# pujariaditya/WaveVerify

Measured on AMD Instinct MI355X. Metric: clips/sec embed+detect, 1s@16kHz bs=256, higher is better.
Workload: dtype f32; 1 GPU; embed_detect: 256 clips x 1 s @ 16 kHz per GPU (BASELINE.json configs[1]), seeded random weights; batch_per_gpu=256, global_batch=256, clip_samples=16000, parallelism=dp1 (independent clip shards, no data-path collective)

## Files before the change

### waveverify_amd/csrc/wv_rb.hip

```cpp
#include <atomic>
#include <string>

#include "wv_dev.h"

namespace wv {

namespace {

template <int NT> struct RbVec;
template <> struct RbVec<4> { typedef f32x4 type; };
template <> struct RbVec<2> { typedef f32x2 type; };

constexpr int RB_OOB = 0x7f000000;
#ifndef RB_CFG64
#define RB_CFG64 RB<64, 2, 4, 2, 1>
#endif
#ifndef RB_CFG96
#define RB_CFG96 RB<96, 4, 2, 3, 3>
#endif
#ifndef RB_CFG128
#define RB_CFG128 RB<128, 2, 4, 2, 4>
#endif
#ifndef RB_CFG192
#define RB_CFG192 RB<192, 2, 2, 3, 2>
#endif
#ifndef RB_PD
#define RB_PD 3
#endif
#ifndef RB_AD
#define RB_AD 3
#endif

#ifdef RB_STAMP
#define RB_T(i) do { const unsigned long long t_ = __builtin_amdgcn_s_memtime(); ph[i] += t_ - tprev; tprev = t_; } while (0)
#else
#define RB_T(i) do {} while (0)
#endif

template <int C_, int NG_, int NT_, int WPS_, int PARTS_>
struct RB {
    static constexpr int C = C_, NG = NG_, NT = NT_, WPS = WPS_, PARTS = PARTS_;
    static constexpr int WM = C / 32, NWAVES = WM * NG, NTHREADS = 64 * NWAVES;
    static constexpr int GS = 32 * NT - 4;
    static constexpr int WD = NG * GS + 4;
    static constexpr int TTO = WD - 8;
    static constexpr int LD = WD;
    static constexpr int NCH = C / 16;
    static constexpr int W4 = WD / 4, P4 = C * W4;
    static constexpr int RPI = 64 / W4;
    static constexpr int NI = (C / RPI + NWAVES - 1) / NWAVES;
    static constexpr size_t SMEM = ((size_t)C * LD + 2 * C * 8) * sizeof(float);
    static_assert(C % 32 == 0 && WD % 4 == 0 && (NT == 2 || NT == 4) && NTHREADS >= 2 * C && RPI >= 1 && C % RPI == 0 && 16 % RPI == 0 &&
                  PARTS >= 1 && NCH % PARTS == 0, "geometry");
    static_assert((2 * NCH) % (RB_AD + 1) == 0, "the A ring must close over a tile");
};

#define RB_BARRIER()                                             \
    do {                                                         \
        asm volatile("s_waitcnt lgkmcnt(0)" ::: "memory");       \
        __builtin_amdgcn_s_barrier();                            \
        asm volatile("" ::: "memory");                           \
    } while (0)

__device__ __forceinline__ float rb_dpp_next(float v) {
    return __builtin_bit_cast(float, __builtin_amdgcn_update_dpp(0, __builtin_bit_cast(int, v), 0x130, 0xf, 0xf, true));
}

__device__ __forceinline__ f32x2 rb_pair_next(f32x2 v) { return f32x2{rb_dpp_next(v.x), rb_dpp_next(v.y)}; }
template <int NT>
__device__ __forceinline__ void rb_stencil2(const f32x16 (&acc)[NT], int r, const float* tp, f32x2 (&y)[NT]) {
    const f32x4 q0 = *reinterpret_cast<const f32x4*>(tp), q1 = *reinterpret_cast<const f32x4*>(tp + 4), q2 = *reinterpret_cast<const f32x4*>(tp + 8);
    const f32x2 w[5] = {{q0.x, q0.y}, {q0.z, q0.w}, {q1.x, q1.y}, {q1.z, q1.w}, {q2.x, q2.y}};
    const f32x2 bb{q2.z, q2.w};
    f32x2 col[NT + 4];
#pragma unroll
    for (int e = 0; e < NT; ++e) col[e] = f32x2{acc[e][r], acc[e][r + 1]};
    if constexpr (NT == 4) {
#pragma unroll
        for (int e = 0; e < 4; ++e) col[4 + e] = rb_pair_next(col[e]);
    } else {
        col[2] = rb_pair_next(col[0]); col[3] = rb_pair_next(col[1]);
        col[4] = rb_pair_next(col[2]); col[5] = rb_pair_next(col[3]);
    }
#pragma unroll
    for (int e = 0; e < NT; ++e) {
        f32x2 v = bb;
#pragma unroll
        for (int i = 0; i < 5; ++i) v = __builtin_elementwise_fma(w[i], col[e + i], v);
        y[e] = v;
    }
}

template <class R, int G0, class LoadA, class AtChunk>
__device__ __forceinline__ void rb_gemm(f32x16 (&acc)[R::NT], f32x4 (&ar)[RB_AD + 1][2], const float* Bf, LoadA&& load_a,
                                        const __amdgpu_buffer_rsrc_t& rw, const __amdgpu_buffer_rsrc_t& rw_next, AtChunk&& at_chunk) {
    typedef typename RbVec<R::NT>::type bvec;
    constexpr int NS = 8 * R::NCH, PD = RB_PD, NB = PD + 1, AD = RB_AD, NA = AD + 1;
    bvec bq[NB];
    auto row_of = [](int s) { return 16 * (s >> 3) + ((s & 7) < 4 ? (s & 7) : 4 + (s & 7)); };
#pragma unroll
    for (int s = 0; s < PD; ++s) bq[s % NB] = *reinterpret_cast<const bvec*>(Bf + row_of(s) * R::LD);
#pragma unroll
    for (int s = 0; s < NS; ++s) {
        const int c = s >> 3, j = s & 7;
        if (j == 0) {
            if (c > 0) at_chunk(c);
            if (c + AD < R::NCH) load_a(rw, c + AD, ar[(G0 + c + AD) % NA]);
            else load_a(rw_next, c + AD - R::NCH, ar[(G0 + c + AD) % NA]);
        }
        if (s + PD < NS) bq[(s + PD) % NB] = *reinterpret_cast<const bvec*>(Bf + row_of(s + PD) * R::LD);
        const f32x4 av = ar[(G0 + c) % NA][j >> 2];
        const float a = av[j & 3];
        const bvec bv = bq[s % NB];
#pragma unroll
        for (int e = 0; e < R::NT; ++e) acc[e] = __builtin_amdgcn_mfma_f32_32x32x2f32(a, bv[e], acc[e], 0, 0, 0);
        __builtin_amdgcn_sched_barrier(0);
    }
}

template <class R, int OUT>
__global__ __launch_bounds__(R::NTHREADS) __attribute__((amdgpu_waves_per_eu(R::WPS, R::WPS))) void rb_kernel(RbArgs p) {
    extern __shared__ __attribute__((aligned(16))) float smem[];
    typedef typename RbVec<R::NT>::type ovec;
    typedef unsigned uvec __attribute__((ext_vector_type(R::NT)));
    constexpr int NT = R::NT, C = R::C, LD = R::LD, NCH = R::NCH, AD = RB_AD, NA = AD + 1;
    float* S = smem;
    float* tab = smem + C * LD;
    const int tid = threadIdx.x, lane = tid & 63;
    const int wave = __builtin_amdgcn_readfirstlane(tid >> 6);
    const int strip = wave % R::WM, grp = wave / R::WM;
    const int h = lane >> 5, q = lane & 31;
    const int T = p.T, ntiles = p.ntiles, num_t = p.num_t;
    const int row_bytes = T * 4, clip_bytes = C * T * 4;

    for (int i = tid; i < C * 8; i += R::NTHREADS) {
        const int m = i >> 3, j = i & 7;
        if (j < 6) {
            const int d = (m >> 1) * 12 + 2 * (j < 5 ? j : 5) + (m & 1);
            tab[d] = p.tab1[i]; tab[C * 8 + d] = p.tab2[i];
        }
    }

    constexpr int MP = (C + M_ALIGN - 1) / M_ALIGN * M_ALIGN;
    const __amdgpu_buffer_rsrc_t rW1 = uniform_rsrc(p.pw1.wq, NCH * 4 * MP * 16);
    const __amdgpu_buffer_rsrc_t rW2 = uniform_rsrc(p.pw2.wq, NCH * 4 * MP * 16);
    const int avoff = (h * MP + 32 * strip + q) * 16;
    f32x4 ar[NA][2];
    auto load_a = [&](const __amdgpu_buffer_rsrc_t& rw, int c, f32x4 (&dst)[2]) {
        dst[0] = __builtin_bit_cast(f32x4, __builtin_amdgcn_raw_buffer_load_b128(rw, avoff, c * 4 * MP * 16, 0));
        dst[1] = __builtin_bit_cast(f32x4, __builtin_amdgcn_raw_buffer_load_b128(rw, avoff, (c * 4 + 2) * MP * 16, 0));
    };

    const int co = R::GS * grp + NT * q;
    const bool own = NT * q < R::GS && co < R::TTO;
    const bool uw = NT * q < R::GS;
    const int row0 = 32 * strip + 4 * h;
    const float* Bf = S + co + 4 * h * LD;
    const float* Wrow1 = tab + (row0 / 2) * 12;
    const float* Wrow2 = Wrow1 + C * 8;
    float* Urow = S + row0 * LD + co;
    float* Xrow = Urow + 8;
    const bool hthread = tid < 2 * C;
    const int hrow = tid >> 1, hpc = tid & 1;

    ovec X[16];
    const int xrow = lane / R::W4, xc4 = lane - xrow * R::W4;
    const bool xlane = lane < R::RPI * R::W4;
    auto refill = [&](int t, int row0_, int row1_) {
        if (t < 0) return;
        const int b = t / num_t, tt = t - b * num_t;
        const int tw0 = tt * R::TTO - 8;
        const __amdgpu_buffer_rsrc_t rX = uniform_rsrc(p.X + (size_t)b * C * T, clip_bytes);
        const int tx = tw0 + 4 * xc4;
        const int vo = (tx >= 0 && tx < T) ? (xrow * T + tx) * 4 : RB_OOB;
        if (xlane) {
#pragma unroll
            for (int i = 0; i < R::NI; ++i) {
                const int rb = i * R::NWAVES + wave;
                const int r_ = rb * R::RPI, so = r_ * row_bytes;
                float* dst = S + r_ * LD;
                if (r_ >= row0_ && r_ < row1_)
                    __builtin_amdgcn_raw_ptr_buffer_load_lds(rX, (__attribute__((address_space(3))) void*)dst, 16, vo, so, 0, 0);
            }
        }
    };
    auto x_off = [&](int to0) { const int t = to0 + co; return (own && t < T) ? (row0 * T + t) * 4 : RB_OOB; };
    const bool h0own = (OUT & 4) && co >= 8 && co < R::WD && (NT * q < R::GS || (grp == R::NG - 1 && NT * q < R::GS + 4));
    const bool u_own = (OUT & 4) && uw && co >= 4 && co < R::WD - 4;
    auto sv_off = [&](bool mine, int t) { return (mine && t < T) ? (row0 * T + t) * 4 : RB_OOB; };
    const float oscale = p.out_scale_ptr ? p.out_scale * p.out_scale_ptr[0] : p.out_scale;

    int tile = blockIdx.x;
    if (tile >= ntiles) return;
    refill(tile, 0, C);
#pragma unroll
    for (int c = 0; c < AD; ++c) load_a(rW1, c, ar[c % NA]);
    asm volatile("s_waitcnt vmcnt(0)" ::: "memory");
    RB_BARRIER();

#ifdef RB_STAMP
    unsigned long long ph[9] = {0, 0, 0, 0, 0, 0, 0, 0, 0}, tprev = __builtin_amdgcn_s_memtime();
#endif
    for (; tile < ntiles; tile += gridDim.x) {
        const int b = tile / num_t, tt = tile - b * num_t;
        const int to0 = tt * R::TTO;
        if (hthread) {
            f32x4* hp = reinterpret_cast<f32x4*>(S + hrow * LD + 4 * hpc);
            f32x4 v = *hp;
            v.x = elu1(v.x * p.pre_scale); v.y = elu1(v.y * p.pre_scale); v.z = elu1(v.z * p.pre_scale); v.w = elu1(v.w * p.pre_scale);
            *hp = v;
        }
        if (own) {
#pragma unroll
            for (int r = 0; r < 16; ++r) X[r] = *reinterpret_cast<const ovec*>(Xrow + ((r & 3) + 8 * (r >> 2)) * LD);
#pragma unroll
            for (int r = 0; r < 16; ++r) {
                ovec v;
#pragma unroll
                for (int e = 0; e < NT; ++e) v[e] = elu1(X[r][e] * p.pre_scale);
                *reinterpret_cast<ovec*>(Xrow + ((r & 3) + 8 * (r >> 2)) * LD) = v;
            }
        }
        RB_T(0);
        RB_BARRIER();
        RB_T(1);
        f32x16 acc[NT];
#pragma unroll
        for (int e = 0; e < NT; ++e)
#pragma unroll
            for (int r = 0; r < 16; ++r) acc[e][r] = 0.f;
        rb_gemm<R, 0>(acc, ar, Bf, load_a, rW1, rW2, [](int) {});
        RB_T(2);
        RB_BARRIER();
        RB_T(3);
        {
            const size_t bo1 = (size_t)b * C * T;
            const __amdgpu_buffer_rsrc_t rH0 = uniform_rsrc((OUT & 4) ? p.sv_h0 + bo1 : p.X, (OUT & 4) ? clip_bytes : 0);
            const __amdgpu_buffer_rsrc_t rU = uniform_rsrc((OUT & 4) ? p.sv_u + bo1 : p.X, (OUT & 4) ? clip_bytes : 0);
            const int vh0 = sv_off(h0own, to0 - 8 + co), vu = sv_off(u_own, to0 - 4 + co);
#pragma unroll
            for (int r = 0; r < 16; r += 2) {
                const int cr = (r & 3) + 8 * (r >> 2);
                f32x2 y2[NT];
                rb_stencil2<NT>(acc, r, Wrow1 + (cr / 2) * 12, y2);
#pragma unroll
                for (int k = 0; k < 2; ++k) {
                    ovec uv;
#pragma unroll
                    for (int e = 0; e < NT; ++e) uv[e] = elu1(y2[e][k] * 1.f);
                    if (uw) *reinterpret_cast<ovec*>(Urow + (cr + k) * LD) = uv;
                    if constexpr ((OUT & 4) != 0) {
                        ovec hv, ur;
#pragma unroll
                        for (int e = 0; e < NT; ++e) { hv[e] = acc[e][r + k]; ur[e] = y2[e][k]; }
                        const int o0 = vh0 == RB_OOB ? RB_OOB : vh0 + (cr + k) * row_bytes, o1 = vu == RB_OOB ? RB_OOB : vu + (cr + k) * row_bytes;
                        if constexpr (NT == 4) {
                            __builtin_amdgcn_raw_buffer_store_b128(__builtin_bit_cast(uvec, hv), rH0, o0, 0, 0);
                            __builtin_amdgcn_raw_buffer_store_b128(__builtin_bit_cast(uvec, ur), rU, o1, 0, 0);
                        } else {
                            __builtin_amdgcn_raw_buffer_store_b64(__builtin_bit_cast(uvec, hv), rH0, o0, 0, 0);
                            __builtin_amdgcn_raw_buffer_store_b64(__builtin_bit_cast(uvec, ur), rU, o1, 0, 0);
                        }
                    }
                }
                __builtin_amdgcn_sched_barrier(0);
            }
            if (tt == 0 && grp == 0 && NT * q < 4) {
                ovec z;
#pragma unroll
                for (int e = 0; e < NT; ++e) z[e] = 0.f;
#pragma unroll
                for (int r = 0; r < 16; ++r) *reinterpret_cast<ovec*>(Urow + ((r & 3) + 8 * (r >> 2)) * LD) = z;
            }
        }
        RB_T(4);
        RB_BARRIER();
        RB_T(5);
#pragma unroll
        for (int e = 0; e < NT; ++e)
#pragma unroll
            for (int r = 0; r < 16; ++r) acc[e][r] = 0.f;
        const int next = tile + gridDim.x < ntiles ? tile + gridDim.x : -1;
        rb_gemm<R, NCH>(acc, ar, Bf, load_a, rW2, rW1, [&](int c) {
            if (R::PARTS > 1 && c % (NCH / R::PARTS) == 0) {
                constexpr int per = NCH / R::PARTS;
                RB_BARRIER();
                refill(next, 16 * (c - per), 16 * c);
            }
        });
        RB_T(6);
        RB_BARRIER();
        RB_T(7);
        {
            const size_t bo = (size_t)b * C * T;
            const __amdgpu_buffer_rsrc_t rY = uniform_rsrc((OUT & 1) ? p.Y + bo : p.X, (OUT & 1) ? clip_bytes : 0);
            const __amdgpu_buffer_rsrc_t rA = uniform_rsrc((OUT & 2) ? p.Yact + bo : p.X, (OUT & 2) ? clip_bytes : 0);
            const int voff0 = x_off(to0);
            const __amdgpu_buffer_rsrc_t rH1 = uniform_rsrc((OUT & 4) ? p.sv_h1 + bo : p.X, (OUT & 4) ? clip_bytes : 0);
            const __amdgpu_buffer_rsrc_t rV = uniform_rsrc((OUT & 4) ? p.sv_v + bo : p.X, (OUT & 4) ? clip_bytes : 0);
            const int vh1 = sv_off(u_own, to0 - 4 + co);
            refill(next, R::PARTS > 1 ? 16 * (NCH - NCH / R::PARTS) : 0, C);
#pragma unroll
            for (int r = 0; r < 16; r += 2) {
                const int cr0 = (r & 3) + 8 * (r >> 2);
                f32x2 v2[NT];
                rb_stencil2<NT>(acc, r, Wrow2 + (cr0 / 2) * 12, v2);
#pragma unroll
                for (int k = 0; k < 2; ++k) {
                    const int cr = cr0 + k;
                    ovec y;
#pragma unroll
                    for (int e = 0; e < NT; ++e) y[e] = fmaf(v2[e][k], oscale, X[r + k][e]);
                    const int off = voff0 + cr * row_bytes;
                    if constexpr ((OUT & 4) != 0) {
                        ovec hv, vv;
#pragma unroll
                        for (int e = 0; e < NT; ++e) { hv[e] = acc[e][r + k]; vv[e] = v2[e][k]; }
                        const int o1 = vh1 == RB_OOB ? RB_OOB : vh1 + cr * row_bytes;
                        if constexpr (NT == 4) {
                            __builtin_amdgcn_raw_buffer_store_b128(__builtin_bit_cast(uvec, hv), rH1, o1, 0, 0);
                            __builtin_amdgcn_raw_buffer_store_b128(__builtin_bit_cast(uvec, vv), rV, off, 0, 0);
                        } else {
                            __builtin_amdgcn_raw_buffer_store_b64(__builtin_bit_cast(uvec, hv), rH1, o1, 0, 0);
                            __builtin_amdgcn_raw_buffer_store_b64(__builtin_bit_cast(uvec, vv), rV, off, 0, 0);
                        }
                    }
                    if constexpr ((OUT & 1) != 0) {
                        if constexpr (NT == 4) __builtin_amdgcn_raw_buffer_store_b128(__builtin_bit_cast(uvec, y), rY, off, 0, 0);
                        else __builtin_amdgcn_raw_buffer_store_b64(__builtin_bit_cast(uvec, y), rY, off, 0, 0);
                    }
                    if constexpr ((OUT & 2) != 0) {
                        ovec a;
#pragma unroll
                        for (int e = 0; e < NT; ++e) a[e] = elu1(y[e] * p.act_scale);
                        if constexpr (NT == 4) __builtin_amdgcn_raw_buffer_store_b128(__builtin_bit_cast(uvec, a), rA, off, 0, 0);
                        else __builtin_amdgcn_raw_buffer_store_b64(__builtin_bit_cast(uvec, a), rA, off, 0, 0);
                    }
                }
                __builtin_amdgcn_sched_barrier(0);
            }
        }
        RB_T(8);
        asm volatile("s_waitcnt vmcnt(%0)" :: "n"(16 * ((OUT & 1) + ((OUT >> 1) & 1) + ((OUT & 4) ? 2 : 0))) : "memory");
        RB_BARRIER();
    }
#ifdef RB_STAMP
    if (lane == 0 && (OUT & 1)) {
        asm volatile("s_waitcnt vmcnt(0)" ::: "memory");
        for (int i = 0; i < 9; ++i) p.Y[((size_t)blockIdx.x * R::NWAVES + wave) * 9 + i] = (float)ph[i];
    }
#endif
}

bool aligned16(const void* p) { return (reinterpret_cast<uintptr_t>(p) & 15) == 0; }

int cu_count() {
    static std::atomic<int> cached[32];
    int d = 0;
    (void)hipGetDevice(&d);
    d &= 31;
    int n = cached[d].load(std::memory_order_relaxed);
    if (n == 0) {
        hipDeviceProp_t pr;
        n = hipGetDeviceProperties(&pr, d) == hipSuccess && pr.multiProcessorCount > 0 ? pr.multiProcessorCount : 256;
        cached[d].store(n, std::memory_order_relaxed);
    }
    return n;
}

template <class R, int OUT>
hipError_t rb_launch(RbArgs a, hipStream_t s) {
    a.num_t = (a.T + R::TTO - 1) / R::TTO;
    const long long nt = (long long)a.num_t * a.B;
    if (nt > 0x7fffffffLL) return hipErrorInvalidValue;
    a.ntiles = (int)nt;
    static std::atomic<unsigned> attr{0};
    if (R::SMEM > 64 * 1024) {
        int d = 0; (void)hipGetDevice(&d);
        const unsigned bit = 1u << (d & 31);
        if (!(attr.load(std::memory_order_relaxed) & bit)) {
            hipError_t e = hipFuncSetAttribute(reinterpret_cast<const void*>(rb_kernel<R, OUT>),
                                               hipFuncAttributeMaxDynamicSharedMemorySize, (int)R::SMEM);
            if (e != hipSuccess) return e;
            attr.fetch_or(bit, std::memory_order_relaxed);
        }
    }
    const int per_cu = std::max(1, std::min((int)(160 * 1024 / R::SMEM), 4 * R::WPS / R::NWAVES));
    const int grid = (int)std::min<long long>(nt, (long long)cu_count() * per_cu);
    std::string name;
    if (prof::enabled()) name = std::string((OUT & 4) ? "resblock_train<" : "resblock<") + std::to_string(R::C) + "," + std::to_string(R::WD) + ">";
    const double C = a.C, Bd = a.B, T = a.T;
    prof::Scope ps(s, name.c_str(), 2.0 * 2.0 * Bd * C * (C * T + 5.0 * T),
                   4.0 * Bd * C * T * (1.0 + ((OUT & 1) ? 1.0 : 0.0) + ((OUT & 2) ? 1.0 : 0.0) + ((OUT & 4) ? 4.0 : 0.0)));
    hipLaunchKernelGGL((rb_kernel<R, OUT>), dim3((unsigned)grid), dim3(R::NTHREADS), R::SMEM, s, a);
    return hipGetLastError();
}

template <class R>
hipError_t rb_pick_out(const RbArgs& a, hipStream_t s) {
    if (a.sv_h0) return rb_launch<R, 5>(a, s);
    if (a.Y && a.Yact) return rb_launch<R, 3>(a, s);
    if (a.Y) return rb_launch<R, 1>(a, s);
    return rb_launch<R, 2>(a, s);
}

}

bool rb_supported(const RbArgs& a) {
    if (!(a.C == 64 || a.C == 96 || a.C == 128 || a.C == 192)) return false;
    if (!a.X || (!a.Y && !a.Yact) || a.T < 4 || (a.T & 3) || a.B < 1 || !a.pw1.wq || !a.pw2.wq || !a.tab1 || !a.tab2) return false;
    if (a.pw1.M != a.C || a.pw1.K != a.C || a.pw2.M != a.C || a.pw2.K != a.C) return false;
    if (a.pw1.Mp != round_up(a.C, M_ALIGN) || a.pw2.Mp != a.pw1.Mp) return false;
    if ((long long)a.C * a.T * 4 >= RB_OOB) return false;
    if (a.sv_h0 || a.sv_u || a.sv_h1 || a.sv_v) {
        if (!a.sv_h0 || !a.sv_u || !a.sv_h1 || !a.sv_v || !a.Y || a.Yact) return false;
        if (!aligned16(a.sv_h0) || !aligned16(a.sv_u) || !aligned16(a.sv_h1) || !aligned16(a.sv_v)) return false;
    }
    return aligned16(a.X) && (!a.Y || aligned16(a.Y)) && (!a.Yact || aligned16(a.Yact));
}

hipError_t launch_resblock(const RbArgs& a, hipStream_t s) {
    if (!rb_supported(a)) return hipErrorNotSupported;
    switch (a.C) {
        case 64: return rb_pick_out<RB_CFG64>(a, s);
        case 96: return rb_pick_out<RB_CFG96>(a, s);
        case 128: return rb_pick_out<RB_CFG128>(a, s);
        default: return rb_pick_out<RB_CFG192>(a, s);
    }
}

}
```

Baseline: 3370 clips/s.

## Add carry-halo resblock kernel for C=96 and C=192 to drop tile overlap

Adds a new resblock kernel variant (RBC) used for the 96- and 192-channel configs. Each block walks consecutive time tiles of a clip and carries the stencil edge columns between tiles and wave groups through small LDS slots, with DPP lane shifts. This replaces recomputing overlapping halo columns. It removes the redundant GEMM and load work on the overlapped columns and allows full-width tiles. In exchange it adds extra barriers, LDS edge buffers and a serial dependency between tiles within a block.

New measurement: 3420 clips/s, median of 6. Within noise of the previous version (+1.5%).

```diff
diff --git a/waveverify_amd/csrc/wv_rb.hip b/waveverify_amd/csrc/wv_rb.hip
--- a/waveverify_amd/csrc/wv_rb.hip
+++ b/waveverify_amd/csrc/wv_rb.hip
@@ -16,13 +16,13 @@
 #define RB_CFG64 RB<64, 2, 4, 2, 1>
 #endif
 #ifndef RB_CFG96
-#define RB_CFG96 RB<96, 4, 2, 3, 3>
+#define RB_CFG96 RBC<96, 4, 2, 3, 3>
 #endif
 #ifndef RB_CFG128
 #define RB_CFG128 RB<128, 2, 4, 2, 4>
 #endif
 #ifndef RB_CFG192
-#define RB_CFG192 RB<192, 2, 2, 3, 2>
+#define RB_CFG192 RBC<192, 2, 2, 3, 2>
 #endif
 #ifndef RB_PD
 #define RB_PD 3
@@ -40,6 +40,7 @@
 template <int C_, int NG_, int NT_, int WPS_, int PARTS_>
 struct RB {
     static constexpr int C = C_, NG = NG_, NT = NT_, WPS = WPS_, PARTS = PARTS_;
+    static constexpr bool CARRY = false;
     static constexpr int WM = C / 32, NWAVES = WM * NG, NTHREADS = 64 * NWAVES;
     static constexpr int GS = 32 * NT - 4;
     static constexpr int WD = NG * GS + 4;
@@ -55,7 +56,27 @@
     static_assert((2 * NCH) % (RB_AD + 1) == 0, "the A ring must close over a tile");
 };
 
-#define RB_BARRIER()                                             \
+template <int C_, int NG_, int NT_, int WPS_, int PARTS_>
+struct RBC {
+    static constexpr int C = C_, NG = NG_, NT = NT_, WPS = WPS_, PARTS = PARTS_;
+    static constexpr bool CARRY = true;
+    static constexpr int WM = C / 32, NWAVES = WM * NG, NTHREADS = 64 * NWAVES;
+    static constexpr int GS = 32 * NT;
+    static constexpr int WD = NG * GS;
+    static constexpr int TTO = WD;
+    static constexpr int LEAD = 8;
+    static constexpr int LD = WD + 4;
+    static constexpr int NCH = C / 16;
+    static constexpr int W4 = WD / 4;
+    static constexpr int NI = (C + NWAVES - 1) / NWAVES;
+    static constexpr int ES = C * 4;
+    static constexpr int NSLOT = NG + 1;
+    static constexpr size_t SMEM = ((size_t)C * LD + 2 * C * 8 + (2 * NSLOT + 1) * ES) * sizeof(float);
+    static_assert(C % 32 == 0 && (NT == 2 || NT == 4) && W4 <= 64 && LD % 4 == 0 && PARTS >= 1 && NCH % PARTS == 0 && SMEM <= 160 * 1024, "geometry");
+    static_assert((2 * NCH) % (RB_AD + 1) == 0, "the A ring must close over a tile");
+};
+
+#define RB_BARRIER()                                            \
     do {                                                         \
         asm volatile("s_waitcnt lgkmcnt(0)" ::: "memory");       \
         __builtin_amdgcn_s_barrier();                            \
@@ -81,6 +102,38 @@
     } else {
         col[2] = rb_pair_next(col[0]); col[3] = rb_pair_next(col[1]);
         col[4] = rb_pair_next(col[2]); col[5] = rb_pair_next(col[3]);
+    }
+#pragma unroll
+    for (int e = 0; e < NT; ++e) {
+        f32x2 v = bb;
+#pragma unroll
+        for (int i = 0; i < 5; ++i) v = __builtin_elementwise_fma(w[i], col[e + i], v);
+        y[e] = v;
+    }
+}
+
+__device__ __forceinline__ float rb_dpp_prev(float v) {
+    return __builtin_bit_cast(float, __builtin_amdgcn_update_dpp(0, __builtin_bit_cast(int, v), 0x138, 0xf, 0xf, true));
+}
+template <int NT>
+__device__ __forceinline__ void rb_stencil2c(const f32x16 (&acc)[NT], int r, const float* tp, const float* ep, bool q0, f32x2 (&y)[NT]) {
+    const f32x4 q0_ = *reinterpret_cast<const f32x4*>(tp), q1 = *reinterpret_cast<const f32x4*>(tp + 4), q2 = *reinterpret_cast<const f32x4*>(tp + 8);
+    const f32x4 ea = *reinterpret_cast<const f32x4*>(ep), eb = *reinterpret_cast<const f32x4*>(ep + 4);
+    const f32x2 w[5] = {{q0_.x, q0_.y}, {q0_.z, q0_.w}, {q1.x, q1.y}, {q1.z, q1.w}, {q2.x, q2.y}};
+    const f32x2 bb{q2.z, q2.w};
+    f32x2 col[NT + 4];
+#pragma unroll
+    for (int e = 0; e < NT; ++e) col[4 + e] = f32x2{acc[e][r], acc[e][r + 1]};
+    auto prev = [&](f32x2 v, int i) {
+        const float sx = rb_dpp_prev(v.x), sy = rb_dpp_prev(v.y);
+        return f32x2{q0 ? ea[i] : sx, q0 ? eb[i] : sy};
+    };
+    if constexpr (NT == 4) {
+#pragma unroll
+        for (int e = 0; e < 4; ++e) col[e] = prev(col[4 + e], e);
+    } else {
+        col[2] = prev(col[4], 2); col[3] = prev(col[5], 3);
+        col[0] = prev(col[2], 0); col[1] = prev(col[3], 1);
     }
 #pragma unroll
     for (int e = 0; e < NT; ++e) {
@@ -352,6 +405,245 @@
 #endif
 }
 
+struct RbWin { int b, tw0, tlo, thi, fresh; };
+
+template <class R, int OUT>
+__global__ __launch_bounds__(R::NTHREADS) __attribute__((amdgpu_waves_per_eu(R::WPS, R::WPS))) void rbc_kernel(RbArgs p) {
+    extern __shared__ __attribute__((aligned(16))) float smem[];
+    typedef typename RbVec<R::NT>::type ovec;
+    typedef unsigned uvec __attribute__((ext_vector_type(R::NT)));
+    constexpr int NT = R::NT, C = R::C, LD = R::LD, NCH = R::NCH, AD = RB_AD, NA = AD + 1, WD = R::WD, NG = R::NG, ES = R::ES;
+    float* S = smem;
+    float* tab = smem + C * LD;
+    float* E1 = tab + 2 * C * 8;
+    float* E2 = E1 + R::NSLOT * ES;
+    float* Z = E2 + R::NSLOT * ES;
+    const int tid = threadIdx.x, lane = tid & 63;
+    const int wave = __builtin_amdgcn_readfirstlane(tid >> 6);
+    const int strip = wave % R::WM, grp = wave / R::WM;
+    const int h = lane >> 5, q = lane & 31;
+    const int T = p.T, ntiles = p.ntiles, num_t = p.num_t;
+    const int row_bytes = T * 4, clip_bytes = C * T * 4;
+
+    for (int i = tid; i < C * 8; i += R::NTHREADS) {
+        const int m = i >> 3, j = i & 7;
+        if (j < 6) {
+            const int d = (m >> 1) * 12 + 2 * (j < 5 ? j : 5) + (m & 1);
+            tab[d] = p.tab1[i]; tab[C * 8 + d] = p.tab2[i];
+        }
+    }
+    for (int i = tid; i < ES; i += R::NTHREADS) Z[i] = 0.f;
+
+    constexpr int MP = (C + M_ALIGN - 1) / M_ALIGN * M_ALIGN;
+    const __amdgpu_buffer_rsrc_t rW1 = uniform_rsrc(p.pw1.wq, NCH * 4 * MP * 16);
+    const __amdgpu_buffer_rsrc_t rW2 = uniform_rsrc(p.pw2.wq, NCH * 4 * MP * 16);
+    const int avoff = (h * MP + 32 * strip + q) * 16;
+    f32x4 ar[NA][2];
+    auto load_a = [&](const __amdgpu_buffer_rsrc_t& rw, int c, f32x4 (&dst)[2]) {
+        dst[0] = __builtin_bit_cast(f32x4, __builtin_amdgcn_raw_buffer_load_b128(rw, avoff, c * 4 * MP * 16, 0));
+        dst[1] = __builtin_bit_cast(f32x4, __builtin_amdgcn_raw_buffer_load_b128(rw, avoff, (c * 4 + 2) * MP * 16, 0));
+    };
+
+    const int co = R::GS * grp + NT * q;
+    const int row0 = 32 * strip + 4 * h;
+    const float* Bf = S + co + 4 * h * LD;
+    const float* Wrow1 = tab + (row0 / 2) * 12;
+    const float* Wrow2 = Wrow1 + C * 8;
+    float* Xrow = S + row0 * LD + co;
+    const bool q0 = q == 0;
+    const bool ewr = NT * q >= R::GS - 4;
+    const int ecol = row0 * 4 + (ewr ? NT * q - (R::GS - 4) : 0);
+    ovec X[16];
+
+    int g = (int)((long long)ntiles * blockIdx.x / gridDim.x);
+    const int g1 = (int)((long long)ntiles * (blockIdx.x + 1) / gridDim.x);
+    if (g >= g1) return;
+    auto open = [&](int& g_) {
+        RbWin w;
+        w.b = g_ / num_t;
+        const int tt = g_ - w.b * num_t, n = min(num_t - tt, g1 - g_);
+        g_ += n;
+        w.tlo = tt * WD; w.tw0 = w.tlo - (tt ? R::LEAD : 0);
+        w.thi = min(T, (tt + n) * WD);
+        w.fresh = 1;
+        return w;
+    };
+    auto advance = [&](const RbWin& w, int& g_) {
+        RbWin n = w;
+        if (w.tw0 + WD < w.thi) { n.tw0 = n.tlo = w.tw0 + WD; n.fresh = 0; }
+        else if (g_ < g1) n = open(g_);
+        else n.b = -1;
+        return n;
+    };
+    const bool xlane = lane < R::W4;
+    auto refill = [&](const RbWin& w, int row0_, int row1_) {
+        if (w.b < 0) return;
+        const __amdgpu_buffer_rsrc_t rX = uniform_rsrc(p.X + (size_t)w.b * C * T, clip_bytes);
+        const int tx = w.tw0 + 4 * lane;
+        const int vo = (tx >= 0 && tx < T) ? tx * 4 : RB_OOB;
+        if (xlane) {
+#pragma unroll
+            for (int i = 0; i < R::NI; ++i) {
+                const int r_ = i * R::NWAVES + wave, so = r_ * row_bytes;
+                float* dst = S + r_ * LD;
+                if (r_ >= row0_ && r_ < row1_)
+                    __builtin_amdgcn_raw_ptr_buffer_load_lds(rX, (__attribute__((address_space(3))) void*)dst, 16, vo, so, 0, 0);
+            }
+        }
+    };
+    const float oscale = p.out_scale_ptr ? p.out_scale * p.out_scale_ptr[0] : p.out_scale;
+
+    RbWin cur = open(g);
+    int par = 0;
+    refill(cur, 0, C);
+#pragma unroll
+    for (int c = 0; c < AD; ++c) load_a(rW1, c, ar[c % NA]);
+    asm volatile("s_waitcnt vmcnt(0)" ::: "memory");
+    RB_BARRIER();
+
+    for (;;) {
+        const RbWin next = advance(cur, g);
+        const int tl = cur.tw0 + co;
+        const int voff0 = (tl >= cur.tlo && tl < cur.thi) ? (row0 * T + tl) * 4 : RB_OOB;
+        const size_t bo = (size_t)cur.b * C * T;
+#pragma unroll
+        for (int r = 0; r < 16; ++r) X[r] = *reinterpret_cast<const ovec*>(Xrow + ((r & 3) + 8 * (r >> 2)) * LD);
+#pragma unroll
+        for (int r = 0; r < 16; ++r) {
+            ovec v;
+#pragma unroll
+            for (int e = 0; e < NT; ++e) v[e] = elu1(X[r][e] * p.pre_scale);
+            *reinterpret_cast<ovec*>(Xrow + ((r & 3) + 8 * (r >> 2)) * LD) = v;
+        }
+        RB_BARRIER();
+        f32x16 acc[NT];
+#pragma unroll
+        for (int e = 0; e < NT; ++e)
+#pragma unroll
+            for (int r = 0; r < 16; ++r) acc[e][r] = 0.f;
+        rb_gemm<R, 0>(acc, ar, Bf, load_a, rW1, rW2, [](int) {});
+        const int wslot = grp < NG - 1 ? grp : NG - 1 + par;
+        const int rslot = NG - 1 + (par ^ 1);
+        if (ewr) {
+            float* ew = E1 + wslot * ES + ecol;
+#pragma unroll
+            for (int r = 0; r < 16; ++r) {
+                ovec v;
+#pragma unroll
+                for (int e = 0; e < NT; ++e) v[e] = acc[e][r];
+                *reinterpret_cast<ovec*>(ew + ((r & 3) + 8 * (r >> 2)) * 4) = v;
+            }
+        }
+        RB_BARRIER();
+        {
+            const __amdgpu_buffer_rsrc_t rH0 = uniform_rsrc((OUT & 4) ? p.sv_h0 + bo : p.X, (OUT & 4) ? clip_bytes : 0);
+            const __amdgpu_buffer_rsrc_t rU = uniform_rsrc((OUT & 4) ? p.sv_u + bo : p.X, (OUT & 4) ? clip_bytes : 0);
+            const float* er = (grp > 0 ? E1 + (grp - 1) * ES : cur.fresh ? Z : E1 + rslot * ES) + row0 * 4;
+#pragma unroll
+            for (int r = 0; r < 16; r += 2) {
+                const int cr = (r & 3) + 8 * (r >> 2);
+                f32x2 y2[NT];
+                rb_stencil2c<NT>(acc, r, Wrow1 + (cr / 2) * 12, er + cr * 4, q0, y2);
+#pragma unroll
+                for (int k = 0; k < 2; ++k) {
+                    ovec uv;
+#pragma unroll
+                    for (int e = 0; e < NT; ++e) uv[e] = elu1(y2[e][k] * 1.f);
+                    *reinterpret_cast<ovec*>(Xrow + (cr + k) * LD) = uv;
+                    if constexpr ((OUT & 4) != 0) {
+                        ovec hv, ur;
+#pragma unroll
+                        for (int e = 0; e < NT; ++e) { hv[e] = acc[e][r + k]; ur[e] = y2[e][k]; }
+                        const int off = voff0 + (cr + k) * row_bytes;
+                        if constexpr (NT == 4) {
+                            __builtin_amdgcn_raw_buffer_store_b128(__builtin_bit_cast(uvec, hv), rH0, off, 0, 0);
+                            __builtin_amdgcn_raw_buffer_store_b128(__builtin_bit_cast(uvec, ur), rU, off, 0, 0);
+                        } else {
+                            __builtin_amdgcn_raw_buffer_store_b64(__builtin_bit_cast(uvec, hv), rH0, off, 0, 0);
+                            __builtin_amdgcn_raw_buffer_store_b64(__builtin_bit_cast(uvec, ur), rU, off, 0, 0);
+                        }
+                    }
+                }
+                __builtin_amdgcn_sched_barrier(0);
+            }
+        }
+        RB_BARRIER();
+#pragma unroll
+        for (int e = 0; e < NT; ++e)
+#pragma unroll
+            for (int r = 0; r < 16; ++r) acc[e][r] = 0.f;
+        rb_gemm<R, NCH>(acc, ar, Bf, load_a, rW2, rW1, [&](int c) {
+            if (R::PARTS > 1 && c % (NCH / R::PARTS) == 0) {
+                constexpr int per = NCH / R::PARTS;
+                RB_BARRIER();
+                refill(next, 16 * (c - per), 16 * c);
+            }
+        });
+        if (ewr) {
+            float* ew = E2 + wslot * ES + ecol;
+#pragma unroll
+            for (int r = 0; r < 16; ++r) {
+                ovec v;
+#pragma unroll
+                for (int e = 0; e < NT; ++e) v[e] = acc[e][r];
+                *reinterpret_cast<ovec*>(ew + ((r & 3) + 8 * (r >> 2)) * 4) = v;
+            }
+        }
+        RB_BARRIER();
+        {
+            const __amdgpu_buffer_rsrc_t rY = uniform_rsrc((OUT & 1) ? p.Y + bo : p.X, (OUT & 1) ? clip_bytes : 0);
+            const __amdgpu_buffer_rsrc_t rA = uniform_rsrc((OUT & 2) ? p.Yact + bo : p.X, (OUT & 2) ? clip_bytes : 0);
+            const __amdgpu_buffer_rsrc_t rH1 = uniform_rsrc((OUT & 4) ? p.sv_h1 + bo : p.X, (OUT & 4) ? clip_bytes : 0);
+            const __amdgpu_buffer_rsrc_t rV = uniform_rsrc((OUT & 4) ? p.sv_v + bo : p.X, (OUT & 4) ? clip_bytes : 0);
+            const float* er = (grp > 0 ? E2 + (grp - 1) * ES : cur.fresh ? Z : E2 + rslot * ES) + row0 * 4;
+            refill(next, R::PARTS > 1 ? 16 * (NCH - NCH / R::PARTS) : 0, C);
+#pragma unroll
+            for (int r = 0; r < 16; r += 2) {
+                const int cr0 = (r & 3) + 8 * (r >> 2);
+                f32x2 v2[NT];
+                rb_stencil2c<NT>(acc, r, Wrow2 + (cr0 / 2) * 12, er + cr0 * 4, q0, v2);
+#pragma unroll
+                for (int k = 0; k < 2; ++k) {
+                    const int cr = cr0 + k;
+                    ovec y;
+#pragma unroll
+                    for (int e = 0; e < NT; ++e) y[e] = fmaf(v2[e][k], oscale, X[r + k][e]);
+                    const int off = voff0 + cr * row_bytes;
+                    if constexpr ((OUT & 4) != 0) {
+                        ovec hv, vv;
+#pragma unroll
+                        for (int e = 0; e < NT; ++e) { hv[e] = acc[e][r + k]; vv[e] = v2[e][k]; }
+                        if constexpr (NT == 4) {
+                            __builtin_amdgcn_raw_buffer_store_b128(__builtin_bit_cast(uvec, hv), rH1, off, 0, 0);
+                            __builtin_amdgcn_raw_buffer_store_b128(__builtin_bit_cast(uvec, vv), rV, off, 0, 0);
+                        } else {
+                            __builtin_amdgcn_raw_buffer_store_b64(__builtin_bit_cast(uvec, hv), rH1, off, 0, 0);
+                            __builtin_amdgcn_raw_buffer_store_b64(__builtin_bit_cast(uvec, vv), rV, off, 0, 0);
+                        }
+                    }
+                    if constexpr ((OUT & 1) != 0) {
+                        if constexpr (NT == 4) __builtin_amdgcn_raw_buffer_store_b128(__builtin_bit_cast(uvec, y), rY, off, 0, 0);
+                        else __builtin_amdgcn_raw_buffer_store_b64(__builtin_bit_cast(uvec, y), rY, off, 0, 0);
+                    }
+                    if constexpr ((OUT & 2) != 0) {
+                        ovec a;
+#pragma unroll
+                        for (int e = 0; e < NT; ++e) a[e] = elu1(y[e] * p.act_scale);
+                        if constexpr (NT == 4) __builtin_amdgcn_raw_buffer_store_b128(__builtin_bit_cast(uvec, a), rA, off, 0, 0);
+                        else __builtin_amdgcn_raw_buffer_store_b64(__builtin_bit_cast(uvec, a), rA, off, 0, 0);
+                    }
+                }
+                __builtin_amdgcn_sched_barrier(0);
+            }
+        }
+        asm volatile("s_waitcnt vmcnt(%0)" :: "n"(16 * ((OUT & 1) + ((OUT >> 1) & 1) + ((OUT & 4) ? 2 : 0))) : "memory");
+        RB_BARRIER();
+        if (next.b < 0) break;
+        cur = next;
+        par ^= 1;
+    }
+}
+
 bool aligned16(const void* p) { return (reinterpret_cast<uintptr_t>(p) & 15) == 0; }
 
 int cu_count() {
@@ -366,6 +658,12 @@
         cached[d].store(n, std::memory_order_relaxed);
     }
     return n;
+}
+
+template <class R, int OUT>
+constexpr auto rb_entry() -> void (*)(RbArgs) {
+    if constexpr (R::CARRY) return rbc_kernel<R, OUT>;
+    else return rb_kernel<R, OUT>;
 }
 
 template <class R, int OUT>
@@ -379,7 +677,7 @@
         int d = 0; (void)hipGetDevice(&d);
         const unsigned bit = 1u << (d & 31);
         if (!(attr.load(std::memory_order_relaxed) & bit)) {
-            hipError_t e = hipFuncSetAttribute(reinterpret_cast<const void*>(rb_kernel<R, OUT>),
+            hipError_t e = hipFuncSetAttribute(reinterpret_cast<const void*>(rb_entry<R, OUT>()),
                                                hipFuncAttributeMaxDynamicSharedMemorySize, (int)R::SMEM);
             if (e != hipSuccess) return e;
             attr.fetch_or(bit, std::memory_order_relaxed);
@@ -392,7 +690,7 @@
     const double C = a.C, Bd = a.B, T = a.T;
     prof::Scope ps(s, name.c_str(), 2.0 * 2.0 * Bd * C * (C * T + 5.0 * T),
                    4.0 * Bd * C * T * (1.0 + ((OUT & 1) ? 1.0 : 0.0) + ((OUT & 2) ? 1.0 : 0.0) + ((OUT & 4) ? 4.0 : 0.0)));
-    hipLaunchKernelGGL((rb_kernel<R, OUT>), dim3((unsigned)grid), dim3(R::NTHREADS), R::SMEM, s, a);
+    hipLaunchKernelGGL((rb_entry<R, OUT>()), dim3((unsigned)grid), dim3(R::NTHREADS), R::SMEM, s, a);
     return hipGetLastError();
 }
 
```
